# yangt1013/SPEINet

Hardware: AMD Instinct MI355X
Metric: deblurred 720p frames/sec (higher is better)
Workload: dtype f16 (correlation top2)

## Files before the change

speinet_amd/csrc/common.h:

```cpp
#pragma once
#include <hip/hip_runtime.h>
#include <stdint.h>
#include <stdio.h>
#include "../../include/speinet_hip.h"

void spei_set_error(const char* fmt, ...);

#define SPEI_REQUIRE(cond, ...)            \
    do {                                   \
        if (!(cond)) {                     \
            spei_set_error(__VA_ARGS__);   \
            return -1;                     \
        }                                  \
    } while (0)

#define SPEI_CHECK_LAUNCH(name)                                                          \
    do {                                                                                 \
        hipError_t e__ = hipGetLastError();                                              \
        if (e__ != hipSuccess) {                                                         \
            spei_set_error("%s: launch failed: %s", name, hipGetErrorString(e__));       \
            return -2;                                                                   \
        }                                                                                \
    } while (0)

// ... 22 lines not shown
#define SPEI_STAMP_CLK(buf, i) do { } while (0)
#define SPEI_STAMP_AT(buf, i, t) do { } while (0)
#endif

template <auto Kernel>
inline void ensure_dyn_lds(size_t lds) {
    static size_t have[32] = {};
    int dev = 0;
    (void)hipGetDevice(&dev);
    if (dev < 0 || dev >= 32 || lds > have[dev]) {
        (void)hipFuncSetAttribute(reinterpret_cast<const void*>(Kernel), hipFuncAttributeMaxDynamicSharedMemorySize, (int)lds);
        if (dev >= 0 && dev < 32) have[dev] = lds;
    }
}

inline int spei_num_cus() {
    static int have[32] = {};
    int dev = 0;
    (void)hipGetDevice(&dev);
    if (dev < 0 || dev >= 32) return 256;
    if (have[dev] == 0) {
        int n = 0;
        if (hipDeviceGetAttribute(&n, hipDeviceAttributeMultiprocessorCount, dev) != hipSuccess || n <= 0) n = 256;
        have[dev] = n;
    }
    return have[dev];
}

__device__ __forceinline__ void spei_stagger_start(int ntiles, int unit) {
    const int G = gridDim.x, b = blockIdx.x;
    const int mine = (ntiles - b + G - 1) / G, most = (ntiles + G - 1) / G;
    const int phase = (mine < most ? 4 : 0) + ((b >> 3) & 3);
    for (int i = 0; i < phase * unit; ++i) __builtin_amdgcn_s_sleep(32);
}

template <int CTRL>
__device__ __forceinline__ float dpp_mov(float v) {
    return __int_as_float(__builtin_amdgcn_update_dpp(0, __float_as_int(v), CTRL, 0xF, 0xF, true));
}
struct OpSum { static __device__ __forceinline__ float f(float a, float b) { return a + b; } };
struct OpMax { static __device__ __forceinline__ float f(float a, float b) { return fmaxf(a, b); } };
template <int M, typename Op>
__device__ __forceinline__ float xor_combine(float v) {
    if constexpr (M == 8) {
        return Op::f(v, dpp_mov<0x128>(v));
    } else if constexpr (M == 16) {
        const auto r = __builtin_amdgcn_permlane16_swap(__float_as_uint(v), __float_as_uint(v), false, false);
        return Op::f(__uint_as_float(r[0]), __uint_as_float(r[1]));
    } else {
        static_assert(M == 32, "xor_combine: M must be 8, 16 or 32");
        const auto r = __builtin_amdgcn_permlane32_swap(__float_as_uint(v), __float_as_uint(v), false, false);
        return Op::f(__uint_as_float(r[0]), __uint_as_float(r[1]));
    }
}
template <typename Op>
__device__ __forceinline__ float wave_allreduce(float v) {
    v = Op::f(v, dpp_mov<0xB1>(v));
    v = Op::f(v, dpp_mov<0x4E>(v));
    v = Op::f(v, dpp_mov<0x141>(v));
    v = Op::f(v, dpp_mov<0x140>(v));
    v = xor_combine<16, Op>(v);
    return xor_combine<32, Op>(v);
}
__device__ __forceinline__ float wave_sum(float v) { return wave_allreduce<OpSum>(v); }
__device__ __forceinline__ float wave_max(float v) { return wave_allreduce<OpMax>(v); }

__device__ __forceinline__ void lds_barrier() { asm volatile("s_waitcnt lgkmcnt(0)\n\ts_barrier" ::: "memory"); }

typedef float f32x16 __attribute__((ext_vector_type(16)));
typedef float f32x4 __attribute__((ext_vector_type(4)));

template <typename T>
struct lpv {
    typedef T x8 __attribute__((ext_vector_type(8)));
    typedef T x4 __attribute__((ext_vector_type(4)));
    typedef T x2 __attribute__((ext_vector_type(2)));
};
__device__ __forceinline__ f32x16 mfma16(lpv<__bf16>::x8 a, lpv<__bf16>::x8 b, f32x16 c) {
    return __builtin_amdgcn_mfma_f32_32x32x16_bf16(a, b, c, 0, 0, 0);
}
__device__ __forceinline__ f32x16 mfma16(lpv<_Float16>::x8 a, lpv<_Float16>::x8 b, f32x16 c) {
    return __builtin_amdgcn_mfma_f32_32x32x16_f16(a, b, c, 0, 0, 0);
}
template <typename LP>
__device__ __forceinline__ LP to_lp(float v) { return (LP)v; }
template <typename LP>
__device__ __forceinline__ typename lpv<LP>::x4 to_lp4(f32x4 v) {
    typename lpv<LP>::x4 h;
    h[0] = to_lp<LP>(v[0]); h[1] = to_lp<LP>(v[1]); h[2] = to_lp<LP>(v[2]); h[3] = to_lp<LP>(v[3]);
    return h;
}
typedef unsigned u32x4 __attribute__((ext_vector_type(4)));

template <int CTRL>
__device__ __forceinline__ float dpp_quad(float v) {
    return __int_as_float(__builtin_amdgcn_update_dpp(0, __float_as_int(v), CTRL, 0xF, 0xF, true));
}
__device__ __forceinline__ void quad_transpose4(float& a0, float& a1, float& a2, float& a3, int t) {
    const bool b0 = t & 1, b1 = t & 2;
    float s = b0 ? a0 : a1, r = dpp_quad<0xB1>(s);
    if (b0) a0 = r; else a1 = r;
    s = b0 ? a2 : a3; r = dpp_quad<0xB1>(s);
    if (b0) a2 = r; else a3 = r;
    s = b1 ? a0 : a2; r = dpp_quad<0x4E>(s);
    if (b1) a0 = r; else a2 = r;
    s = b1 ? a1 : a3; r = dpp_quad<0x4E>(s);
    if (b1) a1 = r; else a3 = r;
}

__device__ __forceinline__ float spei_gray_px(float r, float g, float b) {
    return __fmaf_rn(0.114f, b, __fmaf_rn(0.2989f, r, 0.587f * g)) / 255.0f;
}
```

speinet_amd/csrc/conv3_pipe16.hip:

```cpp
#include "common.h"
#include <type_traits>

namespace {

constexpr int C = 256;
constexpr int TH = 6, TW = 16;
constexpr int SH = TH + 2, SW = TW + 2, SP = SH * SW;
constexpr int PA = 2 * C + 16;
constexpr int SLAB = SP * PA;
constexpr int NSTEP = 9 * 16;
constexpr int RG = 8;

template <int I, int N, typename F>
__device__ __forceinline__ void static_for(F&& f) {
    if constexpr (I < N) {
        f(std::integral_constant<int, I>{});
        static_for<I + 1, N>(f);
    }
}

template <typename LP>
struct C3Params {
    const float* x;
    const LP* wfrag;
    const float* bias;
    const float* res;
    float* out;
    int H, W, batch, tiles_x, tiles_map, ntiles;
    long long* stamps;
};

template <typename LP>
__global__ __launch_bounds__(512) void conv3_pipe_kernel(const C3Params<LP> p) {
    typedef typename lpv<LP>::x8 lp8;
    typedef typename lpv<LP>::x4 lp4;
    extern __shared__ __attribute__((aligned(16))) unsigned char smem[];

    int tid = threadIdx.x;
    const int lane = tid & 63, wave = __builtin_amdgcn_readfirstlane(tid >> 6);
    int fr = lane & 31, fk = lane >> 5;
    int l16 = tid & 15, rsub = tid >> 4;
    const int HW = p.H * p.W;
    const int G = gridDim.x;

    const __amdgpu_buffer_rsrc_t rsw = __builtin_amdgcn_make_buffer_rsrc(const_cast<LP*>(p.wfrag), 0, 9 * C * C * 2, 0x00020000);
    int lane16 = lane * 16;
    const int wbase = wave * NSTEP;
    auto wload = [&](int q, int rot) -> lp8 {
        return __builtin_bit_cast(lp8, __builtin_amdgcn_raw_buffer_load_b128(rsw, lane16, (wbase + (q & ~15) + ((rot + q) & 15)) * 1024, 0));
    };
    float bias = p.bias ? p.bias[wave * 32 + fr] : 0.f;

    f32x4 xr[2][4];
    auto tile_origin = [&](int t, int& bmap, int& y0, int& x0) {
        bmap = __builtin_amdgcn_readfirstlane(t / p.tiles_map);
        const int r = t - bmap * p.tiles_map;
        const int ty = __builtin_amdgcn_readfirstlane(r / p.tiles_x);
        y0 = ty * TH;
        x0 = (r - ty * p.tiles_x) * TW;
    };
    auto stage_load = [&](int t, int ps, int slot) {
        int bmap, y0, x0;
        tile_origin(t, bmap, y0, x0);
        const int sp = min(ps * 32 + rsub, SP - 1);
        const int sy = sp / SW, sx = sp - sy * SW;
        const int gy = min(max(y0 - 1 + sy, 0), p.H - 1), gx = min(max(x0 - 1 + sx, 0), p.W - 1);
        const float* src = p.x + ((size_t)bmap * HW + (size_t)gy * p.W + gx) * C;
#pragma unroll
        for (int j = 0; j < 4; ++j) xr[slot][j] = reinterpret_cast<const f32x4*>(src)[l16 + 16 * j];
    };
    auto stage_write = [&](int t, int ps, int slot, unsigned char* dst, int rb) {
        int bmap, y0, x0;
        tile_origin(t, bmap, y0, x0);
        const int sp = ps * 32 + rsub;
        const int spc = min(sp, SP - 1);
        const int sy = spc / SW, sx = spc - sy * SW;
        const int gy = y0 - 1 + sy, gx = x0 - 1 + sx;
        const bool inside = gy >= 0 && gy < p.H && gx >= 0 && gx < p.W;
        unsigned char* const row = dst + spc * PA;
#pragma unroll
        for (int j = 0; j < 4; ++j) {
            lp4 hv;
#pragma unroll
            for (int e = 0; e < 4; ++e) hv[e] = to_lp<LP>(inside ? xr[slot][j][e] : 0.f);
            *reinterpret_cast<lp4*>(row + (((l16 + 16 * j) * 8 - rb) & 511)) = hv;
        }
        (void)sp;
    };

    int tile = blockIdx.x;
    auto tile_rot = [&](int t) { return (t % p.tiles_map) & 15; };
    int rot = __builtin_amdgcn_readfirstlane(tile_rot(tile));
    lp8 ring[RG];
#pragma unroll
    for (int d = 0; d < RG; ++d) ring[d] = wload(d, rot);
#pragma unroll
    for (int ps = 0; ps < 5; ++ps) {
        stage_load(tile, ps, 0);
        stage_write(tile, ps, 0, smem, rot * 32);
    }
    __builtin_amdgcn_sched_barrier(0);
    lds_barrier();

    int cur = 0;
    int nth = 0;
    for (; tile < p.ntiles; tile += G, ++nth) {
        if (nth == 1) { SPEI_STAMP(p.stamps, 0); SPEI_STAMP_CLK(p.stamps, 8); }
        asm volatile("" : "+v"(tid), "+v"(fr), "+v"(fk), "+v"(l16), "+v"(rsub), "+v"(lane16), "+v"(bias));
        const unsigned char* const sa = smem + (cur ? SLAB : 0);
        unsigned char* const sn = smem + (cur ? 0 : SLAB);
        const int tnx = tile + G;
        const int rotn = __builtin_amdgcn_readfirstlane(tile_rot(tnx));
        const int tnc = tnx < p.ntiles ? tnx : tile;
        int bmap, y0, x0;
        tile_origin(tile, bmap, y0, x0);
        const size_t moff = (size_t)bmap * HW * C;
        const __amdgpu_buffer_rsrc_t rso = __builtin_amdgcn_make_buffer_rsrc(p.out + moff, 0, HW * (C * 4), 0x00020000);
        const __amdgpu_buffer_rsrc_t rsr = __builtin_amdgcn_make_buffer_rsrc(const_cast<float*>(p.res ? p.res + moff : p.out + moff), 0,
                                                                             p.res ? HW * (C * 4) : 0, 0x00020000);
        const int voff = fk * 4096 + fr * 4;
        const int soff0 = (y0 * p.W + x0) * 1024 + wave * 128;

        f32x16 acc[3];
#pragma unroll
        for (int i = 0; i < 3; ++i)
#pragma unroll
            for (int r = 0; r < 16; ++r) acc[i][r] = bias;
        f32x16 res[3];
        int abase[3];
#pragma unroll
        for (int i = 0; i < 3; ++i) abase[i] = ((2 * i + (fr >> 4)) * SW + (fr & 15)) * PA + fk * 16;

        lp8 tn[3];
#pragma unroll
        for (int i = 0; i < 3; ++i) tn[i] = *reinterpret_cast<const lp8*>(sa + abase[i]);
        static_for<0, NSTEP>([&](auto qc) {
            constexpr int q = decltype(qc)::value;
            lp8 tc[3];
#pragma unroll
            for (int i = 0; i < 3; ++i) tc[i] = tn[i];
            if constexpr (q + 1 < NSTEP) {
                constexpr int tap = (q + 1) >> 4, s = (q + 1) & 15;
                constexpr int toff = ((tap / 3) * SW + tap % 3) * PA + s * 32;
#pragma unroll
                for (int i = 0; i < 3; ++i) tn[i] = *reinterpret_cast<const lp8*>(sa + abase[i] + toff);
            }
            const lp8 w = ring[q % RG];
            ring[q % RG] = q + RG < NSTEP ? wload(q + RG, rot) : wload(q + RG - NSTEP, rotn);
            __builtin_amdgcn_sched_barrier(0);
#pragma unroll
            for (int i = 0; i < 3; ++i) acc[i] = mfma16(tc[i], w, acc[i]);
            if (q == 0) { stage_load(tnc, 0, 0); stage_load(tnc, 1, 1); }
            if (q == 40) { stage_write(tnc, 0, 0, sn, rotn * 32); if (nth == 1) { SPEI_STAMP(p.stamps, 1); SPEI_STAMP_CLK(p.stamps, 9); } }
            if (q == 41) stage_write(tnc, 1, 1, sn, rotn * 32);
            if (q == 44) { stage_load(tnc, 2, 0); stage_load(tnc, 3, 1); }
            if (q == 84) { stage_write(tnc, 2, 0, sn, rotn * 32); if (nth == 1) { SPEI_STAMP(p.stamps, 2); SPEI_STAMP_CLK(p.stamps, 10); } }
            if (q == 85) stage_write(tnc, 3, 1, sn, rotn * 32);
            if (q == 88) stage_load(tnc, 4, 0);
            if (q == 124) stage_write(tnc, 4, 0, sn, rotn * 32);
            if (q == 128) {
                if (nth == 1) { SPEI_STAMP(p.stamps, 3); SPEI_STAMP_CLK(p.stamps, 11); }
#pragma unroll
                for (int i = 0; i < 3; ++i)
#pragma unroll
                    for (int r = 0; r < 16; ++r)
                        res[i][r] = __uint_as_float(__builtin_amdgcn_raw_buffer_load_b32(
                            rsr, voff, soff0 + ((2 * i + (r >> 3)) * p.W + 8 * ((r >> 2) & 1) + (r & 3)) * 1024, 0));
            }
#pragma unroll
            for (int i = 0; i < 3; ++i) asm volatile("" : "+v"(acc[i]));
            __builtin_amdgcn_sched_barrier(0);
        });
        if (nth == 1) { SPEI_STAMP(p.stamps, 4); SPEI_STAMP_CLK(p.stamps, 12); }
#pragma unroll
        for (int i = 0; i < 3; ++i)
#pragma unroll
            for (int r = 0; r < 16; ++r)
                __builtin_amdgcn_raw_buffer_store_b32(__float_as_uint(acc[i][r] + res[i][r]), rso, voff,
                                                      soff0 + ((2 * i + (r >> 3)) * p.W + 8 * ((r >> 2) & 1) + (r & 3)) * 1024, 0);
        if (nth == 1) { SPEI_STAMP(p.stamps, 5); SPEI_STAMP_CLK(p.stamps, 13); }
        lds_barrier();
        if (nth == 1) { SPEI_STAMP(p.stamps, 6); SPEI_STAMP_CLK(p.stamps, 14); }
        cur ^= 1;
        rot = rotn;
    }
}

}

template <typename LP>
static int conv3_launch(const float* x, const void* wfrag, const float* bias, const float* res, float* out, int batch, int H, int W,
                        hipStream_t st) {
    C3Params<LP> p;
    p.x = x; p.wfrag = (const LP*)wfrag; p.bias = bias; p.res = res; p.out = out;
    p.H = H; p.W = W; p.batch = batch;
    p.stamps = spei_stamp_buffer();
    p.tiles_x = W / TW; p.tiles_map = p.tiles_x * (H / TH); p.ntiles = p.tiles_map * batch;
    const size_t lds = (size_t)2 * SLAB;
    ensure_dyn_lds<&conv3_pipe_kernel<LP>>(lds);
    const int grid = p.ntiles < spei_num_cus() ? p.ntiles : spei_num_cus();
    hipLaunchKernelGGL((conv3_pipe_kernel<LP>), dim3(grid), dim3(512), lds, st, p);
    SPEI_CHECK_LAUNCH("spei_conv3x3_256_pipe16");
    return 0;
}

extern "C" int spei_conv3x3_256_pipe16(int fmt, const float* x, const void* w_frag, const float* bias, const float* residual, float* out,
                                       int batch, int H, int W, spei_stream_t stream) {
    SPEI_REQUIRE(x && w_frag && out, "spei_conv3x3_256_pipe16: null pointer");
    SPEI_REQUIRE(fmt == SPEI_BF16 || fmt == SPEI_F16, "spei_conv3x3_256_pipe16: fmt=%d", fmt);
    SPEI_REQUIRE(batch >= 1 && H > 0 && W > 0 && H % TH == 0 && W % TW == 0, "spei_conv3x3_256_pipe16: %d maps of %dx%d (height %% 6, width %% 16)",
                 batch, H, W);
    SPEI_REQUIRE((int64_t)H * W <= (1ll << 21), "spei_conv3x3_256_pipe16: map too large for 32-bit byte offsets");
    SPEI_REQUIRE(x != out, "spei_conv3x3_256_pipe16: the input may not alias the output (tiles read their neighbours' pixels)");
    SPEI_REQUIRE(((uintptr_t)x | (uintptr_t)w_frag | (uintptr_t)out | (uintptr_t)residual) % 16 == 0, "spei_conv3x3_256_pipe16: 16-byte alignment required");
    hipStream_t st = (hipStream_t)stream;
    if (fmt == SPEI_F16) return conv3_launch<_Float16>(x, w_frag, bias, residual, out, batch, H, W, st);
    return conv3_launch<__bf16>(x, w_frag, bias, residual, out, batch, H, W, st);
}
```

speinet_amd/ops.py:

```python
from __future__ import annotations

import ctypes as C
from typing import Optional

import torch

from . import _lib
from .pack import BF16, F16, F32, LP_DTYPE, PackedW, fmt_of

ACT_NONE, ACT_RELU, ACT_GELU = 0, 1, 2
CONV, CONV_T = 0, 1

PRECISIONS = ("f32", "bf16x3", "bf16", "f16")
CORR_PRECISIONS = ("bf16x3", "single", "top2")
_CORR_ALIASES = {"bf16": "single", "bf16r": "top2", "f16": "single"}


class FMap:
    __slots__ = ("t", "H", "W", "C", "ld", "off")

    def __init__(self, t: torch.Tensor, H: int, W: int, C_: int, off: int = 0):
        assert t.is_cuda and t.dtype in (torch.float32, torch.bfloat16, torch.float16) and t.is_contiguous() and t.dim() == 2 and t.shape[0] == H * W
        self.t, self.H, self.W, self.C, self.ld, self.off = t, H, W, C_, t.shape[1], off
        assert off + C_ <= self.ld
# ... 246 lines not shown

    def __setattr__(self, k, v):
        raise AttributeError("Ctx is immutable; use replace()")

    def replace(self, **kw) -> "Ctx":
        d = {k: getattr(self, k) for k in self._FIELDS}
        d.update(kw)
        return Ctx(**d)

    def for_stage(self, name: str) -> "Ctx":
        o = self.stage.get(name)
        if o is None and self.split_decode and self.precision == "f16" and name in self.SPLIT_STAGES:
            o = {"precision": "bf16x3", "commute_any": True}
        return self.replace(**o) if o else self

    def _tp(self, t: Optional[torch.Tensor]) -> C.c_void_p:
        if t is None:
            return C.c_void_p(0)
        assert t.is_cuda and t.is_contiguous()
        assert t.device == self.device, f"tensor on {t.device}, call context on {self.device}"
        return C.c_void_p(t.data_ptr())

    def _fp(self, f: Optional[FMap]) -> C.c_void_p:
        if f is None:
            return C.c_void_p(0)
        assert f.t.device == self.device, f"feature map on {f.t.device}, call context on {self.device}"
        return C.c_void_p(f.ptr)

    def _stream(self) -> C.c_void_p:
        assert torch.cuda.current_device() == self.device.index, \
            f"current device cuda:{torch.cuda.current_device()} != call context {self.device}"
        return C.c_void_p(torch.cuda.current_stream(self.device).cuda_stream)

    @property
    def lp16(self) -> bool:
        return self.precision in ("bf16", "f16")

    @property
    def fmt(self) -> int:
        return F16 if self.precision == "f16" else BF16

    def inter_dtype(self) -> torch.dtype:
        return LP_DTYPE[self.fmt] if (self.lp16 and self.use_slab and self.bf16_storage) else torch.float32

    def any_nonzero(self, x: torch.Tensor, flag: torch.Tensor) -> None:
        _lib.check(_lib.lib().spei_any_nonzero(self._tp(x), x.numel(), self._tp(flag), self._stream()), "spei_any_nonzero")

    def rl_prior(self, img: torch.Tensor, iters: int, lam: float = 0.01) -> torch.Tensor:
        c, h, w = img.shape
        out = torch.empty_like(img)
        scratch = torch.empty_like(img)
        _lib.check(_lib.lib().spei_rl_prior(self._tp(img), self._tp(out), self._tp(scratch), c, h, w, iters, lam, self._stream()),
                   "spei_rl_prior")
        return out

    @_family("conv")
    def conv5_in(self, img: torch.Tensor, w: torch.Tensor, b: torch.Tensor, out: Optional[FMap] = None) -> FMap:
        c, h, wd = img.shape
        assert c == 3
        if out is None:
            out = FMap.empty(h, wd, b.numel(), img.device)
        assert (out.H, out.W, out.C, out.ld, out.off) == (h, wd, b.numel(), b.numel(), 0) and not out.lp
        _lib.check(_lib.lib().spei_conv5_in(self._tp(img), self._tp(w), self._tp(b), self._fp(out), h, wd, b.numel(), self._stream()),
                   "spei_conv5_in")
        return out

    @_family("conv")
    def conv5_out(self, f: FMap, w: torch.Tensor, b: torch.Tensor, out: torch.Tensor, w32=None,
                  b32: Optional[torch.Tensor] = None) -> torch.Tensor:
        assert out.shape == (3, f.H, f.W) and out.is_contiguous() and out.dtype == torch.float32
        if self.lp16 and self.use_slab and w32 is not None and f.C == 32:
            _lib.check(_lib.lib().spei_conv5_out_slab16(self.fmt, self._fp(f), f.ld, f.fmt, self._tp(w32.frag(self.fmt)), self._tp(b32),
                                                       self._tp(out), f.H, f.W, self._stream()), "spei_conv5_out_slab16")
            return out
        if f.lp:
            f = FMap(f.t.float(), f.H, f.W, f.C, f.off)
        _lib.check(_lib.lib().spei_conv5_out(self._fp(f), f.ld, self._tp(w), self._tp(b), self._tp(out), f.H, f.W, f.C, self._stream()),
                   "spei_conv5_out")
        return out

    def _conv3_pipe_ok(self, a, w, N: int, ksize: int, stride: int, act: int, residual, out) -> bool:
        return (self.conv3_pipe and self.lp16 and self.use_slab and ksize == 3 and stride == 1 and N == 256 and a.C == 256 and act == ACT_NONE
                and a.H % 6 == 0 and a.W % 16 == 0 and a.H * a.W <= (1 << 21) and a.t.dtype == torch.float32 and getattr(a, "ld", 256) == 256
                and getattr(a, "off", 0) == 0 and getattr(w, "fhi", None) is not None and tuple(w.shape) == (9, 256, 256)
                and (out is None or (out.t.dtype == torch.float32 and getattr(out, "ld", 256) == 256 and getattr(out, "off", 0) == 0
                                     and out.t.data_ptr() != a.t.data_ptr()))
                and (residual is None or (residual.t.dtype == torch.float32 and getattr(residual, "ld", 256) == 256 and getattr(residual, "off", 0) == 0)))

    @_family("conv")
    def igemm(self, a0: FMap, w, bias: Optional[torch.Tensor], N: int, ksize: int = 1, stride: int = 1,
              mode: int = CONV, act: int = ACT_NONE, a1: Optional[FMap] = None, residual: Optional[FMap] = None,
              rowscale: Optional[torch.Tensor] = None, out: Optional[FMap] = None, out_dtype=torch.float32,
              ln_input: bool = False) -> FMap:
        prec = self.precision
        pad = ksize // 2
        if mode == CONV:
            ho, wo = (a0.H + 2 * pad - ksize) // stride + 1, (a0.W + 2 * pad - ksize) // stride + 1
        else:
            ho, wo = a0.H * stride, a0.W * stride
        if out is None:
            out = FMap.empty(ho, wo, N, a0.t.device, out_dtype)
        assert out.H == ho and out.W == wo and out.C == N
        k0, k1 = a0.C, (a1.C if a1 is not None else 0)
        slab = prec != "f32" and self.use_slab and mode == CONV
        assert slab or (mode == CONV_T and self.lp16 and self.use_slab) or not (a0.lp or out.lp), \
            "16-bit activations are only supported by the slab kernel"
        assert a1 is None or a1.t.dtype == a0.t.dtype
        assert residual is None or not residual.lp
        assert all(f.t.dtype in (torch.float32, LP_DTYPE[self.fmt]) for f in (a0, out)), "16-bit tensors must be in the mode's format"
        if torch.is_tensor(w):
            w = PackedW(w, a0.t.device)
        assert not ln_input or (slab and w.fhi is not None), "ln_input is a feature of the slab kernel"
        assert tuple(w.shape) == (ksize * ksize, N, k0 + k1), (tuple(w.shape), ksize, N, k0, k1)
        if a1 is not None:
            assert (a1.H, a1.W) == (a0.H, a0.W)
        if residual is not None:
            assert (residual.H, residual.W, residual.C) == (ho, wo, N)
        if rowscale is not None:
            assert rowscale.numel() == ho * wo
        tp, fp = self._tp, self._fp
        common = (fp(out), out.ld, fp(residual), residual.ld if residual is not None else 0, tp(rowscale), a0.H, a0.W, ho, wo, N,
                  ksize, stride, pad, mode, act, self._stream())
        srcs = (fp(a0), a0.ld, k0, fp(a1), a1.ld if a1 is not None else 0, k1)
        lib = _lib.lib()
        if (mode == CONV and a1 is None and rowscale is None and not ln_input and out_dtype == torch.float32
                and self._conv3_pipe_ok(a0, w, N, ksize, stride, act, residual, out)):
            _lib.check(lib.spei_conv3x3_256_pipe16(self.fmt, fp(a0), tp(w.frag(self.fmt)), tp(bias), fp(residual), fp(out), 1, a0.H, a0.W,
                                                   self._stream()), "spei_conv3x3_256_pipe16")
        elif (self.conv32_ws_available() and mode == CONV and ksize == 5 and stride == 1 and k0 == 32 and N == 32 and a1 is None
                and residual is None and rowscale is None and not ln_input and act in (ACT_NONE, ACT_RELU) and w.fhi is not None
                and (a0.ld, a0.off, out.ld, out.off) == (32, 0, 32, 0) and a0.t.data_ptr() != out.t.data_ptr()):
            _lib.check(lib.spei_conv32_ws16(self.fmt, fp(a0), a0.fmt, tp(w.frag(self.fmt)), tp(bias), fp(out), out.fmt, 1, a0.H, a0.W, act,
                                            self._stream()), "spei_conv32_ws16")
        elif (self.conv64_ws_available() and mode == CONV and ksize == 5 and stride == 1 and k0 == 64 and N == 64 and a1 is None
                and residual is None and rowscale is None and not ln_input and act in (ACT_NONE, ACT_RELU) and w.fhi is not None
                and (a0.ld, a0.off, out.ld, out.off) == (64, 0, 64, 0) and a0.t.data_ptr() != out.t.data_ptr()):
            _lib.check(lib.spei_conv64_ws16(self.fmt, fp(a0), a0.fmt, tp(w.frag(self.fmt)), tp(bias), fp(out), out.fmt, 1, a0.H, a0.W, act,
                                            self._stream()), "spei_conv64_ws16")
        elif (mode == CONV_T and self.lp16 and self.use_slab and ksize == 3 and stride == 2 and a1 is None and residual is None
                and rowscale is None and N % 32 == 0 and k0 % 32 == 0):
            cf = w.convT_class_frags(self.fmt)
            _lib.check(lib.spei_convt2_slab16(self.fmt, fp(a0), a0.ld, k0, a0.fmt, tp(cf[(0, 0)]), tp(cf[(0, 1)]), tp(cf[(1, 0)]),
                                              tp(cf[(1, 1)]), tp(bias), fp(out), out.ld, out.fmt, a0.H, a0.W, N, act,
                                              self._stream()), "spei_convt2_slab16")
        elif (mode == CONV_T and prec == "bf16x3" and self.use_slab and ksize == 3 and stride == 2 and a1 is None and residual is None
                and rowscale is None and N % 32 == 0 and k0 % 32 == 0 and not a0.lp and not out.lp):
            _hi, _lo, ph, pl = w.convT_class_frags_split()
            _lib.check(lib.spei_convt2_slab16x3(fp(a0), a0.ld, k0, ph, pl, tp(bias), fp(out), out.ld, a0.H, a0.W, N, act, self._stream()),
                       "spei_convt2_slab16x3")
        elif prec == "f32":
            _lib.check(lib.spei_igemm_f32(*srcs, tp(w.f32), tp(bias), *common), "spei_igemm_f32")
        elif slab and w.fhi is not None:
            dims = (a0.H * a0.W, 1, ho * wo, 1) if (ksize == 1 and stride == 1) else (a0.H, a0.W, ho, wo)
            _lib.check(lib.spei_conv_slab16(
                self.fmt, *srcs, a0.fmt, tp(w.frag(self.fmt)), tp(w.flo) if prec == "bf16x3" else _vp(0), tp(bias), fp(out), out.ld,
                out.fmt, fp(residual), residual.ld if residual is not None else 0,
                tp(rowscale), *dims, N, ksize, stride, pad, act, int(ln_input), self._stream()), "spei_conv_slab16")
        else:
            assert prec != "f16", "f16: N and K must be multiples of 32 (slab kernel)"
            _lib.check(lib.spei_igemm_bf16(*srcs, tp(w.hi), tp(w.lo) if prec == "bf16x3" else _vp(0), tp(bias), *common),
                       "spei_igemm_bf16")
        return out

    def linear(self, x: torch.Tensor, w, b: Optional[torch.Tensor], act: int = ACT_NONE,
               residual: Optional[torch.Tensor] = None, out: Optional[torch.Tensor] = None, out_dtype=torch.float32,
               ln_input: bool = False) -> torch.Tensor:
        m, k = x.shape
        if torch.is_tensor(w):
            w = PackedW(w.reshape(1, *w.shape), x.device)
        n = w.shape[1]
        if out is None:
            out = torch.empty(m, n, device=x.device, dtype=out_dtype)
        self.igemm(FMap(x, m, 1, k), w, b, n, act=act, ln_input=ln_input,
                   residual=FMap(residual, m, 1, n) if residual is not None else None, out=FMap(out, m, 1, n))
        return out

    @_family("streaming")
    def resblock_gates(self, x1: FMap, pk: dict):
        dev = x1.t.device
        lib = _lib.lib()
        tp = self._tp
        assert x1.off == 0 and x1.ld == x1.C
        s = torch.empty(x1.C, device=dev)
        g1 = torch.empty(x1.H, x1.C, device=dev)
        g2 = torch.empty(x1.W, x1.C, device=dev)
        ws = torch.empty(lib.spei_gate_ws_floats(x1.H, x1.W, x1.C), device=dev)
        _lib.check(lib.spei_resblock_gates(self._fp(x1), x1.fmt, x1.H, x1.W, x1.C, tp(pk["se_w1"]), tp(pk["se_b1"]), tp(pk["se_w2"]),
                                           tp(pk["se_b2"]), tp(pk["cw_w"]), tp(pk["cw_bn"]), tp(pk["hc_w"]), tp(pk["hc_bn"]),
                                           tp(s), tp(g1), tp(g2), tp(ws), self._stream()), "spei_resblock_gates")
        return s, g1, g2

    def apply_fused_available(self, c: int) -> bool:
        return self.lp16 and self.use_slab and self.x1_bf16 and self.fuse_apply and c in (32, 64, 128, 256)

    def resblock(self, x, pk: dict, extra: Optional[FMap] = None, out: Optional[FMap] = None, defer: bool = False):
        idt = self.inter_dtype()
        if isinstance(x, tuple):
            px, px1, ps, pg1, pg2 = x
            c = px.C
            xn = FMap.empty(px.H, px.W, c, px.t.device)
            t = FMap.empty(px.H, px.W, c, px.t.device, idt)
            w1 = pk["w1"] if not torch.is_tensor(pk["w1"]) else PackedW(pk["w1"], px.t.device)
            _lib.check(_lib.lib().spei_conv_slab16_fa(self.fmt, self._fp(px), c, self._fp(px1), self._tp(ps), self._tp(pg1), self._tp(pg2),
                                                      self._fp(xn), self._tp(w1.frag(self.fmt)), self._tp(pk["b1"]), self._fp(t), t.ld, t.fmt,
                                                      px.H, px.W, c, 5, ACT_RELU, self._stream()), "spei_conv_slab16_fa")
            x = xn
        else:
            c = x.C
            assert x.off == 0 and x.ld == c
            t = self.igemm(x, pk["w1"], pk["b1"], c, ksize=5, act=ACT_RELU, out_dtype=idt)
        x1 = self.igemm(t, pk["w2"], pk["b2"], c, ksize=5, out_dtype=idt if self.x1_bf16 else torch.float32)
        s, g1, g2 = self.resblock_gates(x1, pk)
        if defer:
            return (x, x1, s, g1, g2)
        if out is None:
            out = FMap.empty(x.H, x.W, c, x.t.device)
        if extra is not None:
            assert extra.off == 0 and extra.ld == c
        self._apply(x, x1, s, g1, g2, extra, out, c)
        return out

    @_family("streaming")
    def _apply(self, x, x1, s, g1, g2, extra, out, c):
        _lib.check(_lib.lib().spei_resblock_apply(self._fp(x), self._fp(x1), x1.fmt, self._tp(s), self._tp(g1), self._tp(g2),
                                                  self._fp(extra), self._fp(out), out.ld, x.H, x.W, c, self._stream()),
                   "spei_resblock_apply")

    def batched_available(self) -> bool:
        return self.batched_kernels() and self.x1_bf16 and self.bf16_storage and not self.fuse_apply and self.batch_enc

    def conv32_ws_available(self) -> bool:
        return self.lp16 and self.use_slab and self.conv32_ws

    def conv64_ws_available(self) -> bool:
        return self.lp16 and self.use_slab and (self.conv32_ws if self.conv64_ws is None else self.conv64_ws)

    def batched_kernels(self) -> bool:
        return self.lp16 and self.use_slab

    @_family("conv")
    def igemm_batched(self, a: BMap, w, bias: torch.Tensor, N: int, ksize: int, stride: int = 1, act: int = ACT_NONE,
                      out_dtype=torch.float32, residual: Optional[BMap] = None, out: Optional[BMap] = None) -> BMap:
        assert self.batched_kernels() and not torch.is_tensor(w) and w.fhi is not None
        pad = ksize // 2
        ho, wo = (a.H + 2 * pad - ksize) // stride + 1, (a.W + 2 * pad - ksize) // stride + 1
        assert tuple(w.shape) == (ksize * ksize, N, a.C) and a.t.dtype in (torch.float32, LP_DTYPE[self.fmt])
        if out is None:
            out = BMap.empty(a.B, ho, wo, N, a.t.device, out_dtype)
        assert (out.B, out.H, out.W, out.C) == (a.B, ho, wo, N) and out.t.data_ptr() != a.t.data_ptr()
        if residual is not None:
            assert (residual.B, residual.H, residual.W, residual.C) == (a.B, ho, wo, N) and residual.t.dtype == torch.float32
            assert residual.t.data_ptr() != a.t.data_ptr()
        tp = self._tp
        if out_dtype == torch.float32 and self._conv3_pipe_ok(a, w, N, ksize, stride, act, residual, out):
            _lib.check(_lib.lib().spei_conv3x3_256_pipe16(self.fmt, tp(a.t), tp(w.frag(self.fmt)), tp(bias),
                                                          tp(residual.t) if residual is not None else _vp(0), tp(out.t), a.B, a.H, a.W,
                                                          self._stream()), "spei_conv3x3_256_pipe16")
            return out
        if (self.conv32_ws_available() and ksize == 5 and stride == 1 and a.C == 32 and N == 32 and residual is None
                and act in (ACT_NONE, ACT_RELU)):
            _lib.check(_lib.lib().spei_conv32_ws16(self.fmt, tp(a.t), a.fmt, tp(w.frag(self.fmt)), tp(bias), tp(out.t), out.fmt, a.B, a.H, a.W,
                                                   act, self._stream()), "spei_conv32_ws16")
            return out
        if (self.conv64_ws_available() and ksize == 5 and stride == 1 and a.C == 64 and N == 64 and residual is None
                and act in (ACT_NONE, ACT_RELU)):
            _lib.check(_lib.lib().spei_conv64_ws16(self.fmt, tp(a.t), a.fmt, tp(w.frag(self.fmt)), tp(bias), tp(out.t), out.fmt, a.B, a.H, a.W,
                                                   act, self._stream()), "spei_conv64_ws16")
            return out
        _lib.check(_lib.lib().spei_conv_slab16_batched(self.fmt, tp(a.t), a.C, a.fmt, tp(w.frag(self.fmt)), _vp(0), tp(bias), tp(out.t), out.fmt,
                                                       tp(residual.t) if residual is not None else _vp(0), a.B, a.H, a.W, ho, wo, N, ksize,
                                                       stride, pad, act, self._stream()),
                   "spei_conv_slab16_batched")
        return out

    def resblock_batched(self, x: BMap, pk: dict) -> BMap:
        idt = self.inter_dtype()
        c, dev = x.C, x.t.device
        lib = _lib.lib()
        tp = self._tp
        t = self.igemm_batched(x, pk["w1"], pk["b1"], c, 5, act=ACT_RELU, out_dtype=idt)
        x1 = self.igemm_batched(t, pk["w2"], pk["b2"], c, 5, out_dtype=idt)
        del t
        return self._gates_apply_batched(x, x1, pk)

    @_family("streaming")
    def _gates_apply_batched(self, x: BMap, x1: BMap, pk: dict) -> BMap:
        c, dev = x.C, x.t.device
        lib = _lib.lib()
        tp = self._tp
        s = torch.empty(x.B, c, device=dev)
        g1 = torch.empty(x.B, x.H, c, device=dev)
        g2 = torch.empty(x.B, x.W, c, device=dev)
        ws = torch.empty(x.B * lib.spei_gate_ws_floats(x.H, x.W, c), device=dev)
        _lib.check(lib.spei_resblock_gates_batched(tp(x1.t), x1.fmt, x.B, x.H, x.W, c, tp(pk["se_w1"]), tp(pk["se_b1"]), tp(pk["se_w2"]),
                                                   tp(pk["se_b2"]), tp(pk["cw_w"]), tp(pk["cw_bn"]), tp(pk["hc_w"]), tp(pk["hc_bn"]),
                                                   tp(s), tp(g1), tp(g2), tp(ws), self._stream()), "spei_resblock_gates_batched")
        out = BMap.empty(x.B, x.H, x.W, c, dev)
        _lib.check(lib.spei_resblock_apply_batched(tp(x.t), tp(x1.t), x1.fmt, tp(s), tp(g1), tp(g2), tp(out.t), x.B, x.H, x.W, c,
                                                   self._stream()), "spei_resblock_apply_batched")
        return out

    def ln_fused_available(self) -> bool:
        return self.precision != "f32" and self.use_slab

    def attn_fused_available(self) -> bool:
        return self.lp16 and self.use_slab and self.fuse_attn and self.bf16_storage

    def mlp_fused_available(self) -> bool:
        return self.lp16 and self.use_slab and self.fuse_mlp

    def swin_multi_available(self) -> bool:
        return self.attn_fused_available() and self.attn_win4 and self.mlp_fused_available() and self.batched_kernels()

    @_family("swin")
    def attn_fused(self, x: torch.Tensor, yhat: torch.Tensor, bk: dict, H: int, W: int, shift: int, out: torch.Tensor) -> torch.Tensor:
        assert x.shape[0] % (H * W) == 0 and x.shape[1] == 256 and x.dtype == torch.float32 and out.shape == x.shape and out.dtype == torch.float32
        f = self.fmt
        assert yhat.shape == x.shape and yhat.dtype == LP_DTYPE[f]
        tp = self._tp
        batch = x.shape[0] // (H * W)
        if self.attn_win4:
            _lib.check(_lib.lib().spei_attn_win4_16(f, tp(x), tp(out), tp(yhat), tp(bk["wq"].frag(f)), tp(bk["bq"]), tp(bk["wkv"].frag(f)),
                                                    tp(bk["bkv"]), tp(bk["wproj"].frag(f)), tp(bk["bproj"]), tp(bk["relbias"]), batch, H, W,
                                                    shift, self._stream()), "spei_attn_win4_16")
            return out
        assert batch == 1, "the two-window kernel takes one map per launch"
        _lib.check(_lib.lib().spei_attn_fused16(f, tp(x), tp(out), tp(yhat), tp(bk["wq"].frag(f)), tp(bk["bq"]), tp(bk["wkv"].frag(f)),
                                                tp(bk["bkv"]), tp(bk["wproj"].frag(f)), tp(bk["bproj"]), tp(bk["relbias"]), H, W, shift,
                                                self._stream()), "spei_attn_fused16")
        return out

    @_family("swin")
    def mlp_fused(self, x: torch.Tensor, w1, b1: torch.Tensor, w2, b2: torch.Tensor, out: torch.Tensor) -> torch.Tensor:
        assert x.shape[1] == 256 and x.dtype == torch.float32 and out.shape == x.shape and out.dtype == torch.float32
        assert tuple(w1.shape) == (1, 512, 256) and tuple(w2.shape) == (1, 256, 512)
        tp = self._tp
        f = self.fmt
        _lib.check(_lib.lib().spei_mlp_fused16(f, tp(x), tp(out), tp(w1.frag(f)), tp(b1), tp(w2.frag(f)), tp(b2), x.shape[0], self._stream()),
# ... 114 lines not shown
```

speinet_amd/pack.py:

```python
from __future__ import annotations

from typing import Dict

import torch

SD = Dict[str, torch.Tensor]


class GemmW:
    __slots__ = ("t",)

    def __init__(self, t: torch.Tensor):
        self.t = t if t.dim() == 3 else t.reshape(1, *t.shape)


F32, BF16, F16 = 0, 1, 2
LP_DTYPE = {BF16: torch.bfloat16, F16: torch.float16}


def fmt_of(dtype) -> int:
    return {torch.float32: F32, torch.bfloat16: BF16, torch.float16: F16}[dtype]


def _frag(w: torch.Tensor) -> torch.Tensor:
    t, n, k = w.shape
    return w.view(t, n // 32, 32, k // 16, 2, 8).permute(1, 0, 3, 4, 2, 5).contiguous()


class PackedW:
    __slots__ = ("f32", "hi", "lo", "shape", "fhi", "flo", "fh16", "_ct")

    def __init__(self, t: torch.Tensor, device):
        self.f32 = t.detach().to(device=device, dtype=torch.float32).contiguous()
        self.hi = self.f32.to(torch.bfloat16)
        self.lo = (self.f32 - self.hi.float()).to(torch.bfloat16)
        self.shape = tuple(self.f32.shape)
        t, n, k = self.shape
        self.fhi = self.flo = self.fh16 = None
        self._ct = {}
        if n % 32 == 0 and k % 32 == 0:
            self.fhi, self.flo = _frag(self.hi), _frag(self.lo)
            self.fh16 = _frag(self.f32.to(torch.float16))

    def frag(self, fmt: int):
        return self.fh16 if fmt == F16 else self.fhi

    def convT_class_frags(self, fmt: int = BF16) -> dict:
        if fmt not in self._ct:
            assert self.shape[0] == 9
            self._ct[fmt] = self._class_frags(self.f32.to(LP_DTYPE[fmt]))
        return self._ct[fmt]

    @staticmethod
    def _class_frags(src: torch.Tensor) -> dict:
        ct = {}
        for py in (0, 1):
            for px in (0, 1):
                kys, kxs = ([0, 2] if py else [1]), ([0, 2] if px else [1])
                ct[(py, px)] = _frag(torch.stack([src[ky * 3 + kx] for ky in kys for kx in kxs]))
        return ct

    def convT_class_frags_split(self):
        if "split" not in self._ct:
            assert self.shape[0] == 9
            hi, lo = self._class_frags(self.hi), self._class_frags(self.lo)
            order = [(0, 0), (0, 1), (1, 0), (1, 1)]
            import ctypes as C
            ph = (C.c_void_p * 4)(*[hi[k].data_ptr() for k in order])
            pl = (C.c_void_p * 4)(*[lo[k].data_ptr() for k in order])
            self._ct["split"] = (hi, lo, ph, pl)
        return self._ct["split"]


def conv_w(w: torch.Tensor) -> torch.Tensor:
    co, ci, kh, kw = w.shape
    return w.permute(2, 3, 0, 1).reshape(kh * kw, co, ci).contiguous()


def convT_w(w: torch.Tensor) -> torch.Tensor:
    ci, co, kh, kw = w.shape
    return w.permute(2, 3, 1, 0).reshape(kh * kw, co, ci).contiguous()


def G(t: torch.Tensor) -> GemmW:
    return GemmW(t)


def _bn_fold(sd: SD, p: str) -> torch.Tensor:
    scale = sd[p + "weight"].double() / torch.sqrt(sd[p + "running_var"].double() + 1e-5)
    shift = sd[p + "bias"].double() - sd[p + "running_mean"].double() * scale
    return torch.stack((scale.reshape(()), shift.reshape(()))).float()


def resblock(sd: SD, p: str) -> dict:
    return {
        "w1": G(conv_w(sd[p + "main.0.main.0.weight"])), "b1": sd[p + "main.0.main.0.bias"],
        "w2": G(conv_w(sd[p + "main.1.main.0.weight"])), "b2": sd[p + "main.1.main.0.bias"],
        "se_w1": sd[p + "se.fc.0.weight"], "se_b1": sd[p + "se.fc.0.bias"],
        "se_w2": sd[p + "se.fc.2.weight"], "se_b2": sd[p + "se.fc.2.bias"],
        "cw_w": sd[p + "te.cw.conv.conv.weight"].reshape(-1), "cw_bn": _bn_fold(sd, p + "te.cw.conv.bn."),
        "hc_w": sd[p + "te.hc.conv.conv.weight"].reshape(-1), "hc_bn": _bn_fold(sd, p + "te.hc.conv.bn."),
    }


def rel_pos_index(ws: int) -> torch.Tensor:
    c = torch.stack(torch.meshgrid([torch.arange(ws), torch.arange(ws)], indexing="ij")).flatten(1)
    rel = (c[:, :, None] - c[:, None, :]).permute(1, 2, 0).contiguous()
    rel[:, :, 0] += ws - 1
    rel[:, :, 1] += ws - 1
    rel[:, :, 0] *= 2 * ws - 1
    return rel.sum(-1)


def swin_block(sd: SD, p: str, heads: int, ws: int) -> dict:
    g1, b1 = sd[p + "norm1.weight"].double(), sd[p + "norm1.bias"].double()
    g2, b2 = sd[p + "norm2.weight"].double(), sd[p + "norm2.bias"].double()
    wq, bq = sd[p + "attn.qkv_y.weight"].double(), sd[p + "attn.qkv_y.bias"].double()
    wkv, bkv = sd[p + "attn.qkv_x.weight"].double(), sd[p + "attn.qkv_x.bias"].double()
    w1, bb1 = sd[p + "mlp.fc1.weight"].double(), sd[p + "mlp.fc1.bias"].double()
    dim = wq.shape[1]
    scale = (dim // heads) ** -0.5
    n = ws * ws
    idx = rel_pos_index(ws).reshape(-1).to(sd[p + "attn.relative_position_bias_table"].device)
    relb = sd[p + "attn.relative_position_bias_table"][idx].reshape(n, n, heads).permute(2, 0, 1).contiguous()
    return {
        "wq": G((scale * wq * g1[None, :]).float().contiguous()), "bq": (scale * (wq @ b1 + bq)).float(),
        "wkv": G((wkv * g1[None, :]).float().contiguous()), "bkv": (wkv @ b1 + bkv).float(),
        "wproj": G(sd[p + "attn.proj.weight"].contiguous()), "bproj": sd[p + "attn.proj.bias"],
# ... 80 lines not shown
```

Measured before the change: 41.49.

## Switch pipelined 3x3 conv to 16x16x32 MFMA with new weight fragment layout

The 256-channel 3x3 conv kernel moves from 32x32x16 MFMA tiles (three accumulators per wave) to 16x16x32 MFMA tiles, with six spatial rows and two 16-channel output halves per wave. Weights are repacked into a new fragment layout, and the LDS row padding, weight-rotation scheme and residual load/store indexing are updated to match. The aim is a better MFMA shape for this tile, and possibly less LDS bank conflict or more useful issue overlap. In exchange the kernel holds more accumulator registers, issues more LDS A-fragment loads and needs extra packed weight copies.

```diff
diff --git a/speinet_amd/csrc/common.h b/speinet_amd/csrc/common.h
--- a/speinet_amd/csrc/common.h
+++ b/speinet_amd/csrc/common.h
@@ -128,6 +128,12 @@
 __device__ __forceinline__ f32x16 mfma16(lpv<_Float16>::x8 a, lpv<_Float16>::x8 b, f32x16 c) {
     return __builtin_amdgcn_mfma_f32_32x32x16_f16(a, b, c, 0, 0, 0);
 }
+__device__ __forceinline__ f32x4 mfma16x16(lpv<__bf16>::x8 a, lpv<__bf16>::x8 b, f32x4 c) {
+    return __builtin_amdgcn_mfma_f32_16x16x32_bf16(a, b, c, 0, 0, 0);
+}
+__device__ __forceinline__ f32x4 mfma16x16(lpv<_Float16>::x8 a, lpv<_Float16>::x8 b, f32x4 c) {
+    return __builtin_amdgcn_mfma_f32_16x16x32_f16(a, b, c, 0, 0, 0);
+}
 template <typename LP>
 __device__ __forceinline__ LP to_lp(float v) { return (LP)v; }
 template <typename LP>
diff --git a/speinet_amd/csrc/conv3_pipe16.hip b/speinet_amd/csrc/conv3_pipe16.hip
--- a/speinet_amd/csrc/conv3_pipe16.hip
+++ b/speinet_amd/csrc/conv3_pipe16.hip
@@ -6,9 +6,9 @@
 constexpr int C = 256;
 constexpr int TH = 6, TW = 16;
 constexpr int SH = TH + 2, SW = TW + 2, SP = SH * SW;
-constexpr int PA = 2 * C + 16;
+constexpr int PA = 2 * C + 32;
 constexpr int SLAB = SP * PA;
-constexpr int NSTEP = 9 * 16;
+constexpr int NSTEP = 9 * 8 * 2;
 constexpr int RG = 8;
 
 template <int I, int N, typename F>
@@ -38,7 +38,7 @@
 
     int tid = threadIdx.x;
     const int lane = tid & 63, wave = __builtin_amdgcn_readfirstlane(tid >> 6);
-    int fr = lane & 31, fk = lane >> 5;
+    int fr = lane & 15, fk = lane >> 4;
     int l16 = tid & 15, rsub = tid >> 4;
     const int HW = p.H * p.W;
     const int G = gridDim.x;
@@ -47,9 +47,10 @@
     int lane16 = lane * 16;
     const int wbase = wave * NSTEP;
     auto wload = [&](int q, int rot) -> lp8 {
-        return __builtin_bit_cast(lp8, __builtin_amdgcn_raw_buffer_load_b128(rsw, lane16, (wbase + (q & ~15) + ((rot + q) & 15)) * 1024, 0));
-    };
-    float bias = p.bias ? p.bias[wave * 32 + fr] : 0.f;
+        return __builtin_bit_cast(lp8, __builtin_amdgcn_raw_buffer_load_b128(
+                                           rsw, lane16, (wbase + (q & ~15) + ((((q >> 1) + rot) & 7) << 1) + (q & 1)) * 1024, 0));
+    };
+    float bias0 = p.bias ? p.bias[wave * 32 + fr] : 0.f, bias1 = p.bias ? p.bias[wave * 32 + 16 + fr] : 0.f;
 
     f32x4 xr[2][4];
     auto tile_origin = [&](int t, int& bmap, int& y0, int& x0) {
@@ -89,7 +90,7 @@
     };
 
     int tile = blockIdx.x;
-    auto tile_rot = [&](int t) { return (t % p.tiles_map) & 15; };
+    auto tile_rot = [&](int t) { return (t % p.tiles_map) & 7; };
     int rot = __builtin_amdgcn_readfirstlane(tile_rot(tile));
     lp8 ring[RG];
 #pragma unroll
@@ -97,7 +98,7 @@
 #pragma unroll
     for (int ps = 0; ps < 5; ++ps) {
         stage_load(tile, ps, 0);
-        stage_write(tile, ps, 0, smem, rot * 32);
+        stage_write(tile, ps, 0, smem, rot * 64);
     }
     __builtin_amdgcn_sched_barrier(0);
     lds_barrier();
@@ -106,7 +107,7 @@
     int nth = 0;
     for (; tile < p.ntiles; tile += G, ++nth) {
         if (nth == 1) { SPEI_STAMP(p.stamps, 0); SPEI_STAMP_CLK(p.stamps, 8); }
-        asm volatile("" : "+v"(tid), "+v"(fr), "+v"(fk), "+v"(l16), "+v"(rsub), "+v"(lane16), "+v"(bias));
+        asm volatile("" : "+v"(tid), "+v"(fr), "+v"(fk), "+v"(l16), "+v"(rsub), "+v"(lane16), "+v"(bias0), "+v"(bias1));
         const unsigned char* const sa = smem + (cur ? SLAB : 0);
         unsigned char* const sn = smem + (cur ? 0 : SLAB);
         const int tnx = tile + G;
@@ -121,63 +122,72 @@
         const int voff = fk * 4096 + fr * 4;
         const int soff0 = (y0 * p.W + x0) * 1024 + wave * 128;
 
-        f32x16 acc[3];
-#pragma unroll
-        for (int i = 0; i < 3; ++i)
-#pragma unroll
-            for (int r = 0; r < 16; ++r) acc[i][r] = bias;
-        f32x16 res[3];
-        int abase[3];
-#pragma unroll
-        for (int i = 0; i < 3; ++i) abase[i] = ((2 * i + (fr >> 4)) * SW + (fr & 15)) * PA + fk * 16;
-
-        lp8 tn[3];
-#pragma unroll
-        for (int i = 0; i < 3; ++i) tn[i] = *reinterpret_cast<const lp8*>(sa + abase[i]);
+        f32x4 acc[TH][2];
+#pragma unroll
+        for (int b = 0; b < TH; ++b)
+#pragma unroll
+            for (int r = 0; r < 4; ++r) {
+                acc[b][0][r] = bias0;
+                acc[b][1][r] = bias1;
+            }
+        f32x4 res[TH][2];
+        int abase[TH];
+#pragma unroll
+        for (int b = 0; b < TH; ++b) abase[b] = (b * SW + fr) * PA + fk * 16;
+
+        lp8 tn[TH], tc[TH];
+#pragma unroll
+        for (int b = 0; b < TH; ++b) tn[b] = *reinterpret_cast<const lp8*>(sa + abase[b]);
         static_for<0, NSTEP>([&](auto qc) {
             constexpr int q = decltype(qc)::value;
-            lp8 tc[3];
-#pragma unroll
-            for (int i = 0; i < 3; ++i) tc[i] = tn[i];
-            if constexpr (q + 1 < NSTEP) {
-                constexpr int tap = (q + 1) >> 4, s = (q + 1) & 15;
-                constexpr int toff = ((tap / 3) * SW + tap % 3) * PA + s * 32;
-#pragma unroll
-                for (int i = 0; i < 3; ++i) tn[i] = *reinterpret_cast<const lp8*>(sa + abase[i] + toff);
+            constexpr int h = q & 1;
+            if constexpr (h == 0) {
+#pragma unroll
+                for (int b = 0; b < TH; ++b) tc[b] = tn[b];
+                if constexpr (q + 2 < NSTEP) {
+                    constexpr int tap = (q + 2) >> 4, s = ((q + 2) >> 1) & 7;
+                    constexpr int toff = ((tap / 3) * SW + tap % 3) * PA + s * 64;
+#pragma unroll
+                    for (int b = 0; b < TH; ++b) tn[b] = *reinterpret_cast<const lp8*>(sa + abase[b] + toff);
+                }
             }
             const lp8 w = ring[q % RG];
             ring[q % RG] = q + RG < NSTEP ? wload(q + RG, rot) : wload(q + RG - NSTEP, rotn);
             __builtin_amdgcn_sched_barrier(0);
 #pragma unroll
-            for (int i = 0; i < 3; ++i) acc[i] = mfma16(tc[i], w, acc[i]);
+            for (int b = 0; b < TH; ++b) acc[b][h] = mfma16x16(tc[b], w, acc[b][h]);
             if (q == 0) { stage_load(tnc, 0, 0); stage_load(tnc, 1, 1); }
-            if (q == 40) { stage_write(tnc, 0, 0, sn, rotn * 32); if (nth == 1) { SPEI_STAMP(p.stamps, 1); SPEI_STAMP_CLK(p.stamps, 9); } }
-            if (q == 41) stage_write(tnc, 1, 1, sn, rotn * 32);
+            if (q == 40) { stage_write(tnc, 0, 0, sn, rotn * 64); if (nth == 1) { SPEI_STAMP(p.stamps, 1); SPEI_STAMP_CLK(p.stamps, 9); } }
+            if (q == 41) stage_write(tnc, 1, 1, sn, rotn * 64);
             if (q == 44) { stage_load(tnc, 2, 0); stage_load(tnc, 3, 1); }
-            if (q == 84) { stage_write(tnc, 2, 0, sn, rotn * 32); if (nth == 1) { SPEI_STAMP(p.stamps, 2); SPEI_STAMP_CLK(p.stamps, 10); } }
-            if (q == 85) stage_write(tnc, 3, 1, sn, rotn * 32);
+            if (q == 84) { stage_write(tnc, 2, 0, sn, rotn * 64); if (nth == 1) { SPEI_STAMP(p.stamps, 2); SPEI_STAMP_CLK(p.stamps, 10); } }
+            if (q == 85) stage_write(tnc, 3, 1, sn, rotn * 64);
             if (q == 88) stage_load(tnc, 4, 0);
-            if (q == 124) stage_write(tnc, 4, 0, sn, rotn * 32);
+            if (q == 124) stage_write(tnc, 4, 0, sn, rotn * 64);
             if (q == 128) {
                 if (nth == 1) { SPEI_STAMP(p.stamps, 3); SPEI_STAMP_CLK(p.stamps, 11); }
 #pragma unroll
-                for (int i = 0; i < 3; ++i)
-#pragma unroll
-                    for (int r = 0; r < 16; ++r)
-                        res[i][r] = __uint_as_float(__builtin_amdgcn_raw_buffer_load_b32(
-                            rsr, voff, soff0 + ((2 * i + (r >> 3)) * p.W + 8 * ((r >> 2) & 1) + (r & 3)) * 1024, 0));
+                for (int b = 0; b < TH; ++b)
+#pragma unroll
+                    for (int hh = 0; hh < 2; ++hh)
+#pragma unroll
+                        for (int r = 0; r < 4; ++r)
+                            res[b][hh][r] = __uint_as_float(
+                                __builtin_amdgcn_raw_buffer_load_b32(rsr, voff, soff0 + (b * p.W + r) * 1024 + hh * 64, 0));
             }
 #pragma unroll
-            for (int i = 0; i < 3; ++i) asm volatile("" : "+v"(acc[i]));
+            for (int b = 0; b < TH; ++b) asm volatile("" : "+v"(acc[b][h]));
             __builtin_amdgcn_sched_barrier(0);
         });
         if (nth == 1) { SPEI_STAMP(p.stamps, 4); SPEI_STAMP_CLK(p.stamps, 12); }
 #pragma unroll
-        for (int i = 0; i < 3; ++i)
-#pragma unroll
-            for (int r = 0; r < 16; ++r)
-                __builtin_amdgcn_raw_buffer_store_b32(__float_as_uint(acc[i][r] + res[i][r]), rso, voff,
-                                                      soff0 + ((2 * i + (r >> 3)) * p.W + 8 * ((r >> 2) & 1) + (r & 3)) * 1024, 0);
+        for (int b = 0; b < TH; ++b)
+#pragma unroll
+            for (int hh = 0; hh < 2; ++hh)
+#pragma unroll
+                for (int r = 0; r < 4; ++r)
+                    __builtin_amdgcn_raw_buffer_store_b32(__float_as_uint(acc[b][hh][r] + res[b][hh][r]), rso, voff,
+                                                          soff0 + (b * p.W + r) * 1024 + hh * 64, 0);
         if (nth == 1) { SPEI_STAMP(p.stamps, 5); SPEI_STAMP_CLK(p.stamps, 13); }
         lds_barrier();
         if (nth == 1) { SPEI_STAMP(p.stamps, 6); SPEI_STAMP_CLK(p.stamps, 14); }
diff --git a/speinet_amd/ops.py b/speinet_amd/ops.py
--- a/speinet_amd/ops.py
+++ b/speinet_amd/ops.py
@@ -352,7 +352,7 @@
     def _conv3_pipe_ok(self, a, w, N: int, ksize: int, stride: int, act: int, residual, out) -> bool:
         return (self.conv3_pipe and self.lp16 and self.use_slab and ksize == 3 and stride == 1 and N == 256 and a.C == 256 and act == ACT_NONE
                 and a.H % 6 == 0 and a.W % 16 == 0 and a.H * a.W <= (1 << 21) and a.t.dtype == torch.float32 and getattr(a, "ld", 256) == 256
-                and getattr(a, "off", 0) == 0 and getattr(w, "fhi", None) is not None and tuple(w.shape) == (9, 256, 256)
+                and getattr(a, "off", 0) == 0 and getattr(w, "f16hi", None) is not None
                 and (out is None or (out.t.dtype == torch.float32 and getattr(out, "ld", 256) == 256 and getattr(out, "off", 0) == 0
                                      and out.t.data_ptr() != a.t.data_ptr()))
                 and (residual is None or (residual.t.dtype == torch.float32 and getattr(residual, "ld", 256) == 256 and getattr(residual, "off", 0) == 0)))
@@ -395,7 +395,7 @@
         lib = _lib.lib()
         if (mode == CONV and a1 is None and rowscale is None and not ln_input and out_dtype == torch.float32
                 and self._conv3_pipe_ok(a0, w, N, ksize, stride, act, residual, out)):
-            _lib.check(lib.spei_conv3x3_256_pipe16(self.fmt, fp(a0), tp(w.frag(self.fmt)), tp(bias), fp(residual), fp(out), 1, a0.H, a0.W,
+            _lib.check(lib.spei_conv3x3_256_pipe16(self.fmt, fp(a0), tp(w.frag16(self.fmt)), tp(bias), fp(residual), fp(out), 1, a0.H, a0.W,
                                                    self._stream()), "spei_conv3x3_256_pipe16")
         elif (self.conv32_ws_available() and mode == CONV and ksize == 5 and stride == 1 and k0 == 32 and N == 32 and a1 is None
                 and residual is None and rowscale is None and not ln_input and act in (ACT_NONE, ACT_RELU) and w.fhi is not None
@@ -523,7 +523,7 @@
             assert residual.t.data_ptr() != a.t.data_ptr()
         tp = self._tp
         if out_dtype == torch.float32 and self._conv3_pipe_ok(a, w, N, ksize, stride, act, residual, out):
-            _lib.check(_lib.lib().spei_conv3x3_256_pipe16(self.fmt, tp(a.t), tp(w.frag(self.fmt)), tp(bias),
+            _lib.check(_lib.lib().spei_conv3x3_256_pipe16(self.fmt, tp(a.t), tp(w.frag16(self.fmt)), tp(bias),
                                                           tp(residual.t) if residual is not None else _vp(0), tp(out.t), a.B, a.H, a.W,
                                                           self._stream()), "spei_conv3x3_256_pipe16")
             return out
diff --git a/speinet_amd/pack.py b/speinet_amd/pack.py
--- a/speinet_amd/pack.py
+++ b/speinet_amd/pack.py
@@ -27,8 +27,13 @@
     return w.view(t, n // 32, 32, k // 16, 2, 8).permute(1, 0, 3, 4, 2, 5).contiguous()
 
 
+def _frag16(w: torch.Tensor) -> torch.Tensor:
+    t, n, k = w.shape
+    return w.view(t, n // 32, 2, 16, k // 32, 4, 8).permute(1, 0, 4, 2, 5, 3, 6).reshape(n // 32, t, k // 32, 2, 64, 8)
+
+
 class PackedW:
-    __slots__ = ("f32", "hi", "lo", "shape", "fhi", "flo", "fh16", "_ct")
+    __slots__ = ("f32", "hi", "lo", "shape", "fhi", "flo", "fh16", "f16hi", "f16h16", "_ct")
 
     def __init__(self, t: torch.Tensor, device):
         self.f32 = t.detach().to(device=device, dtype=torch.float32).contiguous()
@@ -41,9 +46,15 @@
         if n % 32 == 0 and k % 32 == 0:
             self.fhi, self.flo = _frag(self.hi), _frag(self.lo)
             self.fh16 = _frag(self.f32.to(torch.float16))
+        self.f16hi = self.f16h16 = None
+        if self.shape == (9, 256, 256):
+            self.f16hi, self.f16h16 = _frag16(self.hi), _frag16(self.f32.to(torch.float16))
 
     def frag(self, fmt: int):
         return self.fh16 if fmt == F16 else self.fhi
+
+    def frag16(self, fmt: int):
+        return self.f16h16 if fmt == F16 else self.f16hi
 
     def convT_class_frags(self, fmt: int = BF16) -> dict:
         if fmt not in self._ct:
```

Result: no change. 41.59, median of 6 (+0.2%).
